# facebookresearch/omni3d

Measured on AMD Instinct MI355X. Metric: images/sec train DLA34_FPN b=4/GPU, higher is better.
Workload: dtype f32; 1 GPU; cubercnn_DLA34_FPN train step, batch 4/GPU, synthetic Omni3D 512x512 (8 GT/img), fwd+10 losses+bwd+allreduce+divergence guard+SGD, random-init weights; global_batch=4, image=512x512, parallelism=dp1 (flat-bucket RCCL all-reduce)

## Files before the change

### include/omni3d_hip.h

```cpp
#ifndef OMNI3D_HIP_H
#define OMNI3D_HIP_H

#ifdef __cplusplus
extern "C" {
#endif


int omni_iou_box3d(const float* boxes1, int N, const float* boxes2, int M, const int* valid1, float* vol,
                   float* iou, int* overflow, void* stream);

int omni_iou_box3d_pairs(const float* boxes1, const float* boxes2, const int* idx1, const int* idx2,
                         long long npairs, const int* valid1, float* vol, float* iou, int* overflow,
                         void* stream);

int omni_iou_box3d_pairs_algo(const float* boxes1, const float* boxes2, const int* idx1, const int* idx2,
                              long long npairs, const int* valid1, float* vol, float* iou, int* overflow,
                              int lanes_per_pair, void* stream);

int omni_box3d_validity(const float* boxes, int N, float eps_coplanar, float eps_nonzero, int* valid,
                        int* counts, void* stream);

int omni_nms3d(const float* verts, const float* score, const int* cls, const int* count, int B, int S, float iou_thr,
               int class_agnostic, float eps_coplanar, float eps_nonzero, float* iou, int* keep, int* order, int* new_count,
               int* overflow, void* stream);
// ... 102 lines not shown
                              int pad, int groups, void* stream);

int omni_dwconv_fwd(const float* x, const float* w, float* y, int N, int H, int W, int C, int R, int stride, int pad, void* stream);
int omni_dwconv_dgrad(const float* dy, const float* w, float* dx, int N, int H, int W, int C, int R, int stride, int pad, void* stream);
int omni_dwconv_wgrad(const float* x, const float* dy, float* dw, int N, int H, int W, int C, int R, int stride, int pad, void* stream);

int omni_avgpool2_fwd(const float* x, float* y, int N, int H, int W, int C, void* stream);
int omni_avgpool2_bwd(const float* dy, float* dx, int N, int H, int W, int C, void* stream);

int omni_subsample2_fwd(const float* x, float* y, int N, int H, int W, int C, void* stream);
int omni_subsample2_bwd(const float* dy, float* dx, int N, int H, int W, int C, void* stream);

int omni_upsample2_add(const float* lat, const float* top, float* out, int N, int H, int W, int C,
                       void* stream);
int omni_upsample2_bwd(const float* dout, float* dtop, int N, int H, int W, int C, void* stream);

int omni_wino_out_carry(const float* M, const float* carry, long long ldc, float* y, int N, int H, int W, int K, int tile, void* stream);
int omni_maxpool2_bwd_carry(const float* x, const float* dy, long long lddy, const float* carry, long long ldc, float* dx, int N, int H,
                            int W, int C, void* stream);
int omni_subsample2_bwd_carry(const float* dy, const float* carry, long long ldc, float* dx, int N, int H, int W, int C, void* stream);
int omni_upsample2_bwd_carry(const float* dout, const float* carry, long long ldc, float* dtop, int N, int H, int W, int C,
                             void* stream);

int omni_preprocess(const unsigned char* img, float* out, int N, int H, int W, int PH, int PW, float m0,
                    float m1, float m2, float s0, float s1, float s2, void* stream);
int omni_preprocess_masked(const unsigned char* img, const int* image_hw, float* out, int N, int H, int W, int PH, int PW,
                           float m0, float m1, float m2, float s0, float s1, float s2, void* stream);
int omni_preprocess_multi(const void* const* imgs, const int* image_hw, float* out, int N, int H, int W, int PH, int PW, float m0,
                          float m1, float m2, float s0, float s1, float s2, void* stream);

// ... 300 lines not shown
```

### omni3d_amd/csrc/conv_gemm.hip

```cpp
#include <device_rt.h>
#include "split_reduce.h"

namespace {

constexpr int OMNI_MAX_SRC = 6;
struct ConvP {
    const float* x;
    const float* w;
    const float* bias;
    float* out;
    int N, H, W, C;
    int OH, OW, K;
    int R, S, stride, pad;
    int ldx, ldo, ldw;
    int relu;
    int accumulate;
    int splits;
    long xb, wb, ob;
    float* stats;
    float* ws;
    unsigned* ctr;
    const float* xs[OMNI_MAX_SRC];
    int coff[OMNI_MAX_SRC + 1];
    int nsrc;
};


__device__ __forceinline__ float4 ldg4(const float* p) { return *reinterpret_cast<const float4*>(p); }
__device__ __forceinline__ float4 zero4() { return make_float4(0.f, 0.f, 0.f, 0.f); }
typedef unsigned omni_u4 __attribute__((ext_vector_type(4)));
__device__ __forceinline__ float4 bufld4(omni_rsrc_t r, int voff) {
#ifdef OMNI_HIPEMU
    float4 v = zero4();
    if ((unsigned)voff + 16u <= r.bytes) memcpy(&v, r.base + (unsigned)voff, 16);
    return v;
#else
    const omni_u4 u = __builtin_amdgcn_raw_buffer_load_b128(r, voff, 0, 0);
    return make_float4(__uint_as_float(u.x), __uint_as_float(u.y), __uint_as_float(u.z), __uint_as_float(u.w));
#endif
}


__device__ __forceinline__ void tile_coords(int tiles_m, int tiles_n, int& tm, int& tn) {
    const int nwg = tiles_m * tiles_n;
    int id = blockIdx.x;
    const int q = nwg / 8, r = nwg % 8;
    const int xcd = id % 8, k = id / 8;
    const int swz = (xcd < r ? xcd * (q + 1) : r * (q + 1) + (xcd - r) * q) + k;
    id = (nwg >= 8) ? swz : id;
    if (tiles_n <= 4) {
        tn = id % tiles_n;
        tm = id / tiles_n;
    } else {
        tm = id % tiles_m;
        tn = id / tiles_m;
    }
}

__device__ __forceinline__ int xcd_chunked(int id, int total) {
    if (total < 8) return id;
    const int q = total / 8, r = total % 8, xcd = id % 8, k = id / 8;
    return (xcd < r ? xcd * (q + 1) : r * (q + 1) + (xcd - r) * q) + k;
}

template <int WM, int WN, bool A_KCONTIG, bool B_KCONTIG, int LDA, int LDB, int BKX = 16>
__device__ __forceinline__ void mma_slab(const float* __restrict__ As, const float* __restrict__ Bs, int a_row0,
                                         int b_row0, int lane, f32x16 (&acc)[WM][WN]) {
    const int l31 = lane & 31, h = lane >> 5;
    constexpr int BKP = BKX + 4;
#pragma unroll
    for (int kc = 0; kc < BKX / 8; ++kc) {
        float a[WM][4], b[WN][4];
#pragma unroll
        for (int i = 0; i < WM; ++i) {
            if (A_KCONTIG) {
                const float4 v = *reinterpret_cast<const float4*>(As + (a_row0 + 32 * i + l31) * BKP + 8 * kc + 4 * h);
                a[i][0] = v.x; a[i][1] = v.y; a[i][2] = v.z; a[i][3] = v.w;
            } else {
#pragma unroll
                for (int t = 0; t < 4; ++t) a[i][t] = As[(8 * kc + 4 * h + t) * LDA + a_row0 + 32 * i + l31];
            }
        }
#pragma unroll
        for (int j = 0; j < WN; ++j) {
            if (B_KCONTIG) {
                const float4 v = *reinterpret_cast<const float4*>(Bs + (b_row0 + 32 * j + l31) * BKP + 8 * kc + 4 * h);
                b[j][0] = v.x; b[j][1] = v.y; b[j][2] = v.z; b[j][3] = v.w;
            } else {
#pragma unroll
                for (int t = 0; t < 4; ++t) b[j][t] = Bs[(8 * kc + 4 * h + t) * LDB + b_row0 + 32 * j + l31];
            }
        }
#pragma unroll
        for (int t = 0; t < 4; ++t)
#pragma unroll
            for (int i = 0; i < WM; ++i)
#pragma unroll
                for (int j = 0; j < WN; ++j) acc[i][j] = mfma_32x32x2(a[i][t], b[j][t], acc[i][j]);
    }
}

template <int WM, int WN>
__device__ __forceinline__ void zero_acc(f32x16 (&acc)[WM][WN]) {
#pragma unroll
    for (int i = 0; i < WM; ++i)
#pragma unroll
        for (int j = 0; j < WN; ++j)
#pragma unroll
            for (int r = 0; r < 16; ++r) acc[i][j][r] = 0.f;
}

template <int BM, int BN, int WAVES_M, int WAVES_N, int BKX = 16, int PF = 1>
__global__ void __launch_bounds__(256) conv_fwd_kernel(ConvP p) {
    constexpr int WM = BM / (32 * WAVES_M), WN = BN / (32 * WAVES_N);
    constexpr int BKP = BKX + 4, KQ = BKX / 4;
    constexpr int RPP = 256 / KQ;
    constexpr int AI = (BM + RPP - 1) / RPP, BI = (BN + RPP - 1) / RPP;
    __shared__ __attribute__((aligned(16))) float smem[2 * (BM + BN) * BKP];
    p.x += (long)blockIdx.z * p.xb;
    p.w += (long)blockIdx.z * p.wb;
    p.out += (long)blockIdx.z * p.ob;
    const int tid = threadIdx.x, lane = tid & 63, wave = tid >> 6;
    const int wm = wave / WAVES_N, wn = wave % WAVES_N;
    const int M = p.N * p.OH * p.OW, Kd = p.R * p.S * p.C;
// ... 934 lines not shown
    const int local = id - t.first[j];
    if (local >= t.items[j]) return;
    gemm_tn_pf_body<PF>(t.p[j], t.rps[j], t.splits[j], xcd_chunked(local, t.items[j]));
}

inline bool bad_geom(const ConvP& p) {
    return p.N < 0 || p.H <= 0 || p.W <= 0 || p.C <= 0 || p.K <= 0 || p.R <= 0 || p.S <= 0 || p.stride <= 0 ||
           p.pad < 0 || (p.C & 3) || p.OH != (p.H + 2 * p.pad - p.R) / p.stride + 1 ||
           p.OW != (p.W + 2 * p.pad - p.S) / p.stride + 1;
}

}

extern "C" {


struct DetArgs {
    float* ws;
    long long ws_floats;
    unsigned* ctr;
    int n_ctr;
    long long* plan;
};
constexpr DetArgs NO_DET{};
static inline bool det_fits(const DetArgs& d, long tiles, long splits, long tile_elems) {
    return d.ctr != nullptr && d.ws != nullptr && d.n_ctr >= omni_split_counters(tiles, splits) &&
           d.ws_floats >= omni_split_ws_floats(tiles, splits, tile_elems);
}
static inline void det_plan(const DetArgs& d, long tile, long tiles, long splits, long tile_elems) {
    d.plan[0] = tile; d.plan[1] = splits;
// ... 103 lines not shown
    ConvP p = convp_fwd(x, w, bias, out, N, H, W, C, K, R, S, stride, pad, ldx, ldo, relu);
    if (nblk_out) *nblk_out = 0;
    if (ms != nullptr && attach_sources(p, *ms, 32, true) != OMNI_OK) return OMNI_ERR_ARG;
    if (bad_geom(p) || (ldx & 3) || ldx < C || ldo < K || tile < 0 || tile > 4 || splits_req < 0) return OMNI_ERR_ARG;
    if (splits_req > 1 && ldo != K) return OMNI_ERR_ARG;
    const long M = (long)N * p.OH * p.OW;
    if (M == 0) return OMNI_OK;
    hipStream_t st = (hipStream_t)stream;
    const long Kd = (long)R * S * C;
    if (ms == nullptr && !fits_i32(((long)N * H * W - 1) * ldx + C)) return OMNI_ERR_ARG;
    if (!fits_i32((long)K * Kd)) return OMNI_ERR_ARG;
    const long nslab = (Kd + 31) / 32;
    const long t128 = ((M + 127) / 128) * ((K + 127) / 128);
    const long t64 = ((M + 63) / 64) * ((K + 63) / 64);
    long splits = 1;
    if (tile == 0) {
        if (K > 64 && t128 >= 256) {
            tile = 1;
        } else if (K > 64 && t128 >= 64 && Kd >= 2048 && ldo == K) {
            tile = 1;
            splits = (512 + t128 - 1) / t128;
            if (splits > nslab / 8) splits = nslab / 8;
        } else if (K > 32 && (K > 64 || ((M + 127) / 128) < 256)) {
            tile = 2;
            if (t64 < 512 && nslab >= 16 && ldo == K) {
                splits = (1024 + t64 - 1) / t64;
                if (splits > nslab / 8) splits = nslab / 8;
                if (splits > 32) splits = 32;
            }
        } else {
            tile = K > 32 ? 3 : 4;
        }
        if (splits < 1) splits = 1;
    }
    if (splits_req >= 1) splits = splits_req;
    if (splits > nslab) splits = nslab;
    int bm, bn;
    tile_dims(tile, bm, bn);
    const long tiles = ((M + bm - 1) / bm) * ((K + bn - 1) / bn);
    const DetLaunch dl = det_prologue(det, tile, tiles, splits, (long)bm * bn, out, sizeof(float) * (size_t)M * K, false, st);
    if (dl.step != DET_LAUNCH) return dl.step;
    p.ws = dl.ws; p.ctr = dl.ctr;
    if (stats != nullptr && (splits == 1 || dl.ordered) && bias == nullptr && !relu) {
        const long rows = (M + bm - 1) / bm;
        if (rows <= stats_rows) {
            p.stats = stats;
            if (nblk_out) *nblk_out = (int)rows;
        }
    }
#define OMNI_FWD(BM_, BN_, WM_, WN_, BK_, PF_)                                                                           \
    hipLaunchKernelGGL(HIP_KERNEL_NAME(conv_fwd_kernel<BM_, BN_, WM_, WN_, BK_, PF_>), dim3((unsigned)tiles, (unsigned)splits), dim3(256), 0, st, p)
// ... 46 lines not shown
static int conv2d_dgrad_impl(const float* dy, const float* w, float* dx, int N, int H, int W, int C, int K, int R, int S,
                             int stride, int pad, int lddy, int lddx, int accumulate, int tile, int splits_req, void* stream,
                             const DetArgs& det) {
    ConvP p = convp_dgrad(dy, w, dx, N, H, W, C, K, R, S, stride, pad, lddy, lddx, accumulate);
    if (bad_geom(p) || (K & 3) || (lddy & 3) || lddy < K || lddx < C || tile < 0 || tile > 4 || splits_req < 0) return OMNI_ERR_ARG;
    if (splits_req > 1 && lddx != C && !accumulate) return OMNI_ERR_ARG;
    if ((long)N * H * W == 0) return OMNI_OK;
    hipStream_t st = (hipStream_t)stream;
    const unsigned ncls = (unsigned)(stride * stride);
    const long M = (long)N * ((H + stride - 1) / stride) * ((W + stride - 1) / stride);
    const long Kd = (long)((R + stride - 1) / stride) * ((S + stride - 1) / stride) * K;
    const long nslab = (Kd + 31) / 32;
    const long t128 = ((M + 127) / 128) * ((C + 127) / 128);
    const long t64 = ((M + 63) / 64) * ((C + 63) / 64);
    long splits = 1;
    if (tile == 0) {
        if (C > 64 && t128 * ncls >= 256) {
            tile = 1;
        } else if (C > 32 && (C > 64 || ((M + 127) / 128) * ncls < 256)) {
            tile = 2;
            if (t64 * ncls < 512 && nslab >= 16 && (lddx == C || accumulate)) {
                splits = (1024 + t64 * ncls - 1) / (t64 * ncls);
                if (splits > nslab / 8) splits = nslab / 8;
                if (splits > 32) splits = 32;
                if (splits < 1) splits = 1;
            }
        } else {
            tile = C > 32 ? 3 : 4;
        }
    }
    if (splits_req >= 1) splits = splits_req;
    if (splits > nslab) splits = nslab;
    int bm, bn;
    tile_dims(tile, bm, bn);
    const long class_tiles = ((M + bm - 1) / bm) * ((C + bn - 1) / bn);
    const long tiles = class_tiles * ncls;
    const DetLaunch dl = det_prologue(det, tile, tiles, splits, (long)bm * bn, dx, sizeof(float) * (size_t)N * H * W * C, accumulate != 0, st);
    if (dl.step != DET_LAUNCH) return dl.step;
    p.ws = dl.ws; p.ctr = dl.ctr;
    const bool dpf = fits_i32((long)N * p.OH * p.OW * lddy, PF_HEADROOM) && fits_i32((long)K * R * S * C, PF_HEADROOM);
#define OMNI_DGRAD(BM_, BN_, WM_, WN_, BK_, PF_)                                                                         \
    hipLaunchKernelGGL(HIP_KERNEL_NAME(conv_dgrad_kernel<BM_, BN_, WM_, WN_, BK_, PF_>), dim3((unsigned)class_tiles, (unsigned)splits, ncls), dim3(256), 0, st, p)
    if (dpf && tile == 1) OMNI_DGRAD(128, 128, 2, 2, 32, 2);
    else if (dpf && tile == 2) OMNI_DGRAD(64, 64, 2, 2, 32, 2);
    else if (dpf && tile == 3) OMNI_DGRAD(128, 64, 2, 2, 32, 2);
    else if (tile == 1) OMNI_DGRAD(128, 128, 2, 2, 32, 1);
    else if (tile == 2) OMNI_DGRAD(64, 64, 2, 2, 32, 1);
// ... 295 lines not shown
```

### omni3d_amd/cubercnn/modeling/backbone/fpn.py

```python
import math

from torch import nn

from .... import functional as HF
from ....d2.layers import ShapeSpec
from ..layers import Conv2d


class Backbone(nn.Module):
    @property
    def size_divisibility(self):
        return 0

    def output_shape(self):
        return {name: ShapeSpec(channels=self._out_feature_channels[name], stride=self._out_feature_strides[name])
                for name in self._out_features}


class LastLevelMaxPool(nn.Module):

    def __init__(self):
        super().__init__()
        self.num_levels = 1
        self.in_feature = "p5"
# ... 29 lines not shown
            for s in range(stage, stage + top_block.num_levels):
                self._out_feature_strides[f"p{s + 1}"] = 2 ** (s + 1)
        self._out_features = list(self._out_feature_strides.keys())
        self._out_feature_channels = {k: out_channels for k in self._out_features}
        self._size_divisibility = strides[-1]

    @property
    def size_divisibility(self):
        return self._size_divisibility

    def forward(self, x):
        feats = self.bottom_up(x)
        results = {}
        prev = None
        for f, stage in zip(reversed(self.in_features), reversed(self._stages)):
            lat = getattr(self, f"fpn_lateral{stage}")(feats[f])
            prev = lat if prev is None else HF.upsample2_add(lat, prev)
            HF.fanout(prev)
            results[f"p{stage}"] = HF.fanout(getattr(self, f"fpn_output{stage}")(prev))
        if self.top_block is not None:
            src = feats[self.top_block.in_feature] if self.top_block.in_feature in feats else results[self.top_block.in_feature]
            for i, t in enumerate(self.top_block(src)):
                results[f"p{self._stages[-1] + 1 + i}"] = t
        return {k: results[k] for k in self._out_features}
```

### omni3d_amd/functional.py

```python
import torch
from torch.autograd import Function
from os import environ as _environ

_os_environ_get = _environ.get

from .kernels import glue
from .kernels import bnpool, conv, det, wino

CL = torch.channels_last


def _cl(t):
    return t if t.is_contiguous(memory_format=CL) else t.contiguous(memory_format=CL)


def _direct_grad(t):
    if t is not None and getattr(t, "_omni_direct_grad", False) and t.grad is not None and t.requires_grad:
        return t.grad
    return None


def _parts_out(parts, like):
    return parts if parts is not None else like.new_zeros((0, 1))

# ... 640 lines not shown
    def forward(ctx, lat, top):
        ctx.slot = _slot_enter(top, ctx.needs_input_grad[1])
        return bnpool.upsample2_add(_cl(lat), _cl(top))

    @staticmethod
    def backward(ctx, dout):
        dout = _cl(dout)

        def run(carry):
            if carry is not None and _carry_pitch(carry) is None:
                return bnpool.upsample2_bwd(dout) + carry
            return bnpool.upsample2_bwd(dout, carry=carry)
        return dout, _slot_deliver(ctx.slot, run)


class _CatChannels(Function):

    @staticmethod
    def forward(ctx, *xs):
        ctx.slots = [_slot_enter(x, ctx.needs_input_grad[i]) for i, x in enumerate(xs)]
        ctx.sizes = [x.shape[1] for x in xs]
        return torch.cat(xs, 1)

    @staticmethod
    def backward(ctx, g):
        outs, off = [], 0
        for i, (slot, c) in enumerate(zip(ctx.slots, ctx.sizes)):
            piece = g[:, off:off + c]
            off += c
            outs.append(_slot_deliver(slot, lambda carry, piece=piece: _add_carry(piece, carry)) if ctx.needs_input_grad[i] else None)
# ... 82 lines not shown

def max_pool2(x):
    return _MaxPool2.apply(x)


def avg_pool2(x):
    return _AvgPool2.apply(x)


def subsample2(x):
    return _Subsample2.apply(x)


def upsample2_add(lat, top):
    return _Upsample2Add.apply(lat, top)


def _pool_enter(ctx, k, feats):
    ctx.slots = [_slot_enter(f, ctx.needs_input_grad[k + i]) for i, f in enumerate(feats)]
    feats = [_cl(f) for f in feats]
    nhwc = [f.permute(0, 2, 3, 1) for f in feats]
    ctx.shapes = [tuple(f.shape) for f in nhwc]
    return nhwc


def _pool_deliver(ctx, k, dfe):
    return (None,) * k + tuple(_slot_deliver(slot, lambda carry, d=d: _add_carry(d.permute(0, 3, 1, 2), carry)) for slot, d in zip(ctx.slots, dfe))


class _ROIAlign(Function):
# ... 295 lines not shown
```

### omni3d_amd/kernels/conv.py

```python

import torch

from .. import lib as _lib
from . import detmode as _det


def _nhwc(t):
    if t.dim() != 4:
        raise ValueError("expected a 4-D tensor")
    v = t.permute(0, 2, 3, 1)
    if not v.is_contiguous():
        v = v.contiguous()
    return v


def to_channels_last(t):
    return t.contiguous(memory_format=torch.channels_last)


def _fwd_launch(L, x, w, bias, out, N, H, W, C, K, R, S, stride, pad, ldx, ldo, relu, tile, splits, like, stats=None, stats_rows=0, nblk_addr=None):
    if _det.on():
        _det.plan_launch(L, "omni_conv2d_fwd_det", like, (x, w, bias, out, N, H, W, C, K, R, S, stride, pad, ldx, ldo, int(relu)),
                         ask=(tile, splits), late=(_lib.ptr(stats), stats_rows, nblk_addr))
    elif stats is not None:
# ... 81 lines not shown
    n = len(xv)
    ptrs = (ctypes.c_void_p * n)(*[t.data_ptr() for t in xv])
    cs = (ctypes.c_int * n)(*[int(t.shape[3]) for t in xv])
    pa, ca = ctypes.cast(ptrs, ctypes.c_void_p), ctypes.cast(cs, ctypes.c_void_p)
    stats = _stats_buf(K, out.device) if want_stats and bias is None and not relu else None
    cell, addr = _nblk_cell()
    head = (pa, ca, n, _lib.ptr(wv), _lib.ptr(bias), _lib.ptr(out), N, H, W, K, K, int(relu))
    late = (_lib.ptr(stats), STATS_ROWS if stats is not None else 0, addr)
    if _det.on():
        _det.plan_launch(L, "omni_conv2d_fwd_multi_det", xv[0], head, ask=(tile, splits), late=late)
    else:
        L.call("omni_conv2d_fwd_multi_det", *head, tile, splits, *late, None, 0, None, 0, None, _lib.stream_of(xv[0]))
    return out.permute(0, 3, 1, 2), (stats[:cell.value] if stats is not None and cell.value > 0 else None)


def stem_conv_fwd_stats(x, w):
    xv, wv = _nhwc(x), _nhwc(w)
    N, H, W, C = xv.shape
    K, R = wv.shape[0], wv.shape[1]
    L = _lib.check_device(xv, wv)
    out = torch.empty((N, H, W, K), dtype=torch.float32, device=x.device)
    stats = _stats_buf(K, x.device)
    cell, addr = _nblk_cell()
    L.call("omni_stem_conv_fwd_stats", _lib.ptr(xv), _lib.ptr(wv), _lib.ptr(out), N, H, W, C, K, R, C, K, _lib.ptr(stats), STATS_ROWS, addr,
           _lib.stream_of(x))
    return out.permute(0, 3, 1, 2), (stats[:cell.value] if cell.value > 0 else None)


_S2_DGRAD_MIN_WGS = 192

# ... 292 lines not shown
```

### omni3d_amd/profile_io.py

```python
import csv
import hashlib
import os
import re

ROOT = os.path.dirname(os.path.dirname(os.path.abspath(__file__)))


def profile_counters(csv_name, kernel_substr, grid=None):
    path = os.path.join(ROOT, "profiles", csv_name)
    if not os.path.exists(path):
        return None
    digest = hashlib.sha256(open(path, "rb").read()).hexdigest()[:16]
    rows = [r for r in csv.DictReader(open(path)) if kernel_substr in r["kernel"] and (grid is None or int(float(r["grid"])) == grid)]
    if not rows:
        return None
    r = max(rows, key=lambda q: float(q.get("GRBM_GUI_ACTIVE", "0") or 0))

    def f(k):
        try:
            v = float(r[k])
            return v if v == v else None
        except (KeyError, ValueError):
            return None
    out = {"source": f"profiles/{csv_name}", "sha256_16": digest, "kernel": r["kernel"], "grid": int(float(r["grid"]))}
# ... 65 lines not shown
        return None
    if name in VALU_ENTRIES:
        return "valu"
    if name.startswith("omni_rpn_head16"):
        return "head16"
    if name.startswith("omni_stem_conv"):
        return "stem"
    if name.startswith("omni_gemm_engine"):
        return "engine"
    if name == "omni_gemm_batched_wgrad_multi":
        return "gemm_batched_multi"
    if name.startswith("omni_gemm_batched"):
        return "gemm_batched"
    if name.startswith("omni_grouped_conv2d"):
        return "grouped"
    if name in ("omni_conv2d_fwd_multi_det", "omni_conv2d_wgrad_multi_det"):
        return "conv_multi"
    if name == "omni_conv2d_s2_dgrad":
        return "conv_s2"
    if name.startswith("omni_conv2d"):
        return "conv"
    return None


def _host_ints(ptr, n, ctype):
    import ctypes
    if ptr is None:
        return []
    addr = ptr.value if hasattr(ptr, "value") else int(ptr)
    return list(ctypes.cast(addr, ctypes.POINTER(ctype))[:n])


def executed_flops(name, a):
    import ctypes
    cls = flop_class(name)
    if cls in (None, "valu"):
        return 0.0
    v = dict(zip(abi_signatures()[name], a))
    if v.get("plan") is not None:
        return 0.0
    if cls in ("conv", "grouped"):
        OH = (v["H"] + 2 * v["pad"] - v["R"]) // v["stride"] + 1
        OW = (v["W"] + 2 * v["pad"] - v["S"]) // v["stride"] + 1
        return 2.0 * v["N"] * OH * OW * v["K"] * v["R"] * v["S"] * v["C"] / (v["groups"] if cls == "grouped" else 1)
    if cls == "conv_multi":
        return 2.0 * v["N"] * v["H"] * v["W"] * v["K"] * sum(_host_ints(v["cs"], v["nsrc"], ctypes.c_int))
    if cls == "conv_s2":
        return 2.0 * v["N"] * ((v["H"] - 1) // 2 + 1) * ((v["W"] - 1) // 2 + 1) * v["K"] * 9 * v["C"]
    if cls == "stem":
        stride = 2 if "_s2_" in name else 1
        OH, OW = (v["H"] - 1) // stride + 1, (v["W"] - 1) // stride + 1
        return 2.0 * v["N"] * OH * OW * v["K"] * v["R"] * v["R"] * v["C"]
    if cls == "gemm_batched":
        if "N" in v and "C" not in v:
            return 2.0 * v["batch"] * v["M"] * v["N"] * v["K"]
        return 2.0 * v["batch"] * v["M"] * v["C"] * v["K"]
    if cls == "gemm_batched_multi":
        n = v["n"]
        cols = [_host_ints(v[k], n, ctypes.c_int) for k in ("batch", "M", "C", "K")]
        return float(sum(2.0 * b * m * c * k for b, m, c, k in zip(*cols)))
    if cls == "engine":
# ... 81 lines not shown
```

Baseline: 384.0 images/s.

## Add persistent pointwise 1x1 conv GEMM kernel and fuse FPN lateral with upsample-add

Adds a dedicated persistent 1x1-conv GEMM kernel that keeps the full weight slab in shared memory and streams pixel tiles, dispatched automatically for large-M 1x1 forward and dgrad convolutions. The FPN top-down path now fuses the lateral 1x1 conv with the nearest-upsample-and-add of the coarser level in one kernel's epilogue, removing an intermediate tensor write and read. Shared GEMM fragment helpers are moved into a header. The change risks being slower than the tuned generic conv GEMM for some shapes and adds new backward plumbing for the fused op.

```diff
diff --git a/include/omni3d_hip.h b/include/omni3d_hip.h
--- a/include/omni3d_hip.h
+++ b/include/omni3d_hip.h
@@ -140,6 +140,14 @@
 int omni_upsample2_add(const float* lat, const float* top, float* out, int N, int H, int W, int C,
                        void* stream);
 int omni_upsample2_bwd(const float* dout, float* dtop, int N, int H, int W, int C, void* stream);
+
+int omni_conv1x1_fwd_up2add(const float* x, const float* w, const float* bias, const float* top, float* out, int N,
+                            int H, int W, int C, int K, int ldx, int ldo, void* stream);
+int omni_conv1x1_fwd_algo(const void* const* xs, const int* cs, int nsrc, const float* w, const float* bias,
+                          const float* top, float* out, int N, int H, int W, int K, int ldx, int ldo, int relu,
+                          float* stats, int stats_rows, int* nblk_out, int workgroups, void* stream);
+int omni_conv1x1_dgrad_algo(const float* dy, const float* w, float* dx, int N, int H, int W, int C, int K, int lddy,
+                            int lddx, int accumulate, int workgroups, void* stream);
 
 int omni_wino_out_carry(const float* M, const float* carry, long long ldc, float* y, int N, int H, int W, int K, int tile, void* stream);
 int omni_maxpool2_bwd_carry(const float* x, const float* dy, long long lddy, const float* carry, long long ldc, float* dx, int N, int H,
diff --git a/omni3d_amd/csrc/conv_gemm.hip b/omni3d_amd/csrc/conv_gemm.hip
--- a/omni3d_amd/csrc/conv_gemm.hip
+++ b/omni3d_amd/csrc/conv_gemm.hip
@@ -1,5 +1,7 @@
 #include <device_rt.h>
+#include "gemm_frag.h"
 #include "split_reduce.h"
+#include "pointwise_plan.h"
 
 namespace {
 
@@ -26,21 +28,6 @@
 };
 
 
-__device__ __forceinline__ float4 ldg4(const float* p) { return *reinterpret_cast<const float4*>(p); }
-__device__ __forceinline__ float4 zero4() { return make_float4(0.f, 0.f, 0.f, 0.f); }
-typedef unsigned omni_u4 __attribute__((ext_vector_type(4)));
-__device__ __forceinline__ float4 bufld4(omni_rsrc_t r, int voff) {
-#ifdef OMNI_HIPEMU
-    float4 v = zero4();
-    if ((unsigned)voff + 16u <= r.bytes) memcpy(&v, r.base + (unsigned)voff, 16);
-    return v;
-#else
-    const omni_u4 u = __builtin_amdgcn_raw_buffer_load_b128(r, voff, 0, 0);
-    return make_float4(__uint_as_float(u.x), __uint_as_float(u.y), __uint_as_float(u.z), __uint_as_float(u.w));
-#endif
-}
-
-
 __device__ __forceinline__ void tile_coords(int tiles_m, int tiles_n, int& tm, int& tn) {
     const int nwg = tiles_m * tiles_n;
     int id = blockIdx.x;
@@ -55,59 +42,6 @@
         tm = id % tiles_m;
         tn = id / tiles_m;
     }
-}
-
-__device__ __forceinline__ int xcd_chunked(int id, int total) {
-    if (total < 8) return id;
-    const int q = total / 8, r = total % 8, xcd = id % 8, k = id / 8;
-    return (xcd < r ? xcd * (q + 1) : r * (q + 1) + (xcd - r) * q) + k;
-}
-
-template <int WM, int WN, bool A_KCONTIG, bool B_KCONTIG, int LDA, int LDB, int BKX = 16>
-__device__ __forceinline__ void mma_slab(const float* __restrict__ As, const float* __restrict__ Bs, int a_row0,
-                                         int b_row0, int lane, f32x16 (&acc)[WM][WN]) {
-    const int l31 = lane & 31, h = lane >> 5;
-    constexpr int BKP = BKX + 4;
-#pragma unroll
-    for (int kc = 0; kc < BKX / 8; ++kc) {
-        float a[WM][4], b[WN][4];
-#pragma unroll
-        for (int i = 0; i < WM; ++i) {
-            if (A_KCONTIG) {
-                const float4 v = *reinterpret_cast<const float4*>(As + (a_row0 + 32 * i + l31) * BKP + 8 * kc + 4 * h);
-                a[i][0] = v.x; a[i][1] = v.y; a[i][2] = v.z; a[i][3] = v.w;
-            } else {
-#pragma unroll
-                for (int t = 0; t < 4; ++t) a[i][t] = As[(8 * kc + 4 * h + t) * LDA + a_row0 + 32 * i + l31];
-            }
-        }
-#pragma unroll
-        for (int j = 0; j < WN; ++j) {
-            if (B_KCONTIG) {
-                const float4 v = *reinterpret_cast<const float4*>(Bs + (b_row0 + 32 * j + l31) * BKP + 8 * kc + 4 * h);
-                b[j][0] = v.x; b[j][1] = v.y; b[j][2] = v.z; b[j][3] = v.w;
-            } else {
-#pragma unroll
-                for (int t = 0; t < 4; ++t) b[j][t] = Bs[(8 * kc + 4 * h + t) * LDB + b_row0 + 32 * j + l31];
-            }
-        }
-#pragma unroll
-        for (int t = 0; t < 4; ++t)
-#pragma unroll
-            for (int i = 0; i < WM; ++i)
-#pragma unroll
-                for (int j = 0; j < WN; ++j) acc[i][j] = mfma_32x32x2(a[i][t], b[j][t], acc[i][j]);
-    }
-}
-
-template <int WM, int WN>
-__device__ __forceinline__ void zero_acc(f32x16 (&acc)[WM][WN]) {
-#pragma unroll
-    for (int i = 0; i < WM; ++i)
-#pragma unroll
-        for (int j = 0; j < WN; ++j)
-#pragma unroll
-            for (int r = 0; r < 16; ++r) acc[i][j][r] = 0.f;
 }
 
 template <int BM, int BN, int WAVES_M, int WAVES_N, int BKX = 16, int PF = 1>
@@ -1072,6 +1006,12 @@
 
 extern "C" {
 
+int omni_conv1x1_fwd_algo(const void* const* xs, const int* cs, int nsrc, const float* w, const float* bias, const float* top, float* out,
+                          int N, int H, int W, int K, int ldx, int ldo, int relu, float* stats, int stats_rows, int* nblk_out,
+                          int workgroups, void* stream);
+int omni_conv1x1_dgrad_algo(const float* dy, const float* w, float* dx, int N, int H, int W, int C, int K, int lddy, int lddx,
+                            int accumulate, int workgroups, void* stream);
+
 
 struct DetArgs {
     float* ws;
@@ -1205,6 +1145,7 @@
     const long t128 = ((M + 127) / 128) * ((K + 127) / 128);
     const long t64 = ((M + 63) / 64) * ((K + 63) / 64);
     long splits = 1;
+    const bool own_choice = tile == 0 && splits_req == 0;
     if (tile == 0) {
         if (K > 64 && t128 >= 256) {
             tile = 1;
@@ -1226,6 +1167,12 @@
     }
     if (splits_req >= 1) splits = splits_req;
     if (splits > nslab) splits = nslab;
+    if (own_choice && splits == 1 && det.plan == nullptr && R == 1 && S == 1 && stride == 1 && pad == 0 && stats == nullptr && ms == nullptr &&
+        pw_dispatch(M, C)) {
+        const void* xs1[1] = {x};
+        const int cs1[1] = {C};
+        return omni_conv1x1_fwd_algo(xs1, cs1, 1, w, bias, nullptr, out, N, H, W, K, ldx, ldo, relu, nullptr, 0, nullptr, 0, stream);
+    }
     int bm, bn;
     tile_dims(tile, bm, bn);
     const long tiles = ((M + bm - 1) / bm) * ((K + bn - 1) / bn);
@@ -1302,6 +1249,7 @@
     const long t128 = ((M + 127) / 128) * ((C + 127) / 128);
     const long t64 = ((M + 63) / 64) * ((C + 63) / 64);
     long splits = 1;
+    const bool own_choice = tile == 0 && splits_req == 0;
     if (tile == 0) {
         if (C > 64 && t128 * ncls >= 256) {
             tile = 1;
@@ -1319,6 +1267,8 @@
     }
     if (splits_req >= 1) splits = splits_req;
     if (splits > nslab) splits = nslab;
+    if (own_choice && splits == 1 && det.plan == nullptr && R == 1 && S == 1 && stride == 1 && pad == 0 && pw_dispatch(M, K))
+        return omni_conv1x1_dgrad_algo(dy, w, dx, N, H, W, C, K, lddy, lddx, accumulate, 0, stream);
     int bm, bn;
     tile_dims(tile, bm, bn);
     const long class_tiles = ((M + bm - 1) / bm) * ((C + bn - 1) / bn);
diff --git a/omni3d_amd/csrc/gemm_frag.h b/omni3d_amd/csrc/gemm_frag.h
--- /dev/null
+++ b/omni3d_amd/csrc/gemm_frag.h
@@ -0,0 +1,73 @@
+#pragma once
+#include <device_rt.h>
+
+namespace {
+
+__device__ __forceinline__ float4 ldg4(const float* p) { return *reinterpret_cast<const float4*>(p); }
+__device__ __forceinline__ float4 zero4() { return make_float4(0.f, 0.f, 0.f, 0.f); }
+typedef unsigned omni_u4 __attribute__((ext_vector_type(4)));
+__device__ __forceinline__ float4 bufld4(omni_rsrc_t r, int voff) {
+#ifdef OMNI_HIPEMU
+    float4 v = zero4();
+    if ((unsigned)voff + 16u <= r.bytes) memcpy(&v, r.base + (unsigned)voff, 16);
+    return v;
+#else
+    const omni_u4 u = __builtin_amdgcn_raw_buffer_load_b128(r, voff, 0, 0);
+    return make_float4(__uint_as_float(u.x), __uint_as_float(u.y), __uint_as_float(u.z), __uint_as_float(u.w));
+#endif
+}
+
+__device__ __forceinline__ int xcd_chunked(int id, int total) {
+    if (total < 8) return id;
+    const int q = total / 8, r = total % 8, xcd = id % 8, k = id / 8;
+    return (xcd < r ? xcd * (q + 1) : r * (q + 1) + (xcd - r) * q) + k;
+}
+
+template <int WM, int WN, bool A_KCONTIG, bool B_KCONTIG, int LDA, int LDB, int BKX = 16>
+__device__ __forceinline__ void mma_slab(const float* __restrict__ As, const float* __restrict__ Bs, int a_row0,
+                                         int b_row0, int lane, f32x16 (&acc)[WM][WN]) {
+    const int l31 = lane & 31, h = lane >> 5;
+    constexpr int BKP = BKX + 4;
+#pragma unroll
+    for (int kc = 0; kc < BKX / 8; ++kc) {
+        float a[WM][4], b[WN][4];
+#pragma unroll
+        for (int i = 0; i < WM; ++i) {
+            if (A_KCONTIG) {
+                const float4 v = *reinterpret_cast<const float4*>(As + (a_row0 + 32 * i + l31) * BKP + 8 * kc + 4 * h);
+                a[i][0] = v.x; a[i][1] = v.y; a[i][2] = v.z; a[i][3] = v.w;
+            } else {
+#pragma unroll
+                for (int t = 0; t < 4; ++t) a[i][t] = As[(8 * kc + 4 * h + t) * LDA + a_row0 + 32 * i + l31];
+            }
+        }
+#pragma unroll
+        for (int j = 0; j < WN; ++j) {
+            if (B_KCONTIG) {
+                const float4 v = *reinterpret_cast<const float4*>(Bs + (b_row0 + 32 * j + l31) * BKP + 8 * kc + 4 * h);
+                b[j][0] = v.x; b[j][1] = v.y; b[j][2] = v.z; b[j][3] = v.w;
+            } else {
+#pragma unroll
+                for (int t = 0; t < 4; ++t) b[j][t] = Bs[(8 * kc + 4 * h + t) * LDB + b_row0 + 32 * j + l31];
+            }
+        }
+#pragma unroll
+        for (int t = 0; t < 4; ++t)
+#pragma unroll
+            for (int i = 0; i < WM; ++i)
+#pragma unroll
+                for (int j = 0; j < WN; ++j) acc[i][j] = mfma_32x32x2(a[i][t], b[j][t], acc[i][j]);
+    }
+}
+
+template <int WM, int WN>
+__device__ __forceinline__ void zero_acc(f32x16 (&acc)[WM][WN]) {
+#pragma unroll
+    for (int i = 0; i < WM; ++i)
+#pragma unroll
+        for (int j = 0; j < WN; ++j)
+#pragma unroll
+            for (int r = 0; r < 16; ++r) acc[i][j][r] = 0.f;
+}
+
+}
diff --git a/omni3d_amd/csrc/pointwise.hip b/omni3d_amd/csrc/pointwise.hip
--- /dev/null
+++ b/omni3d_amd/csrc/pointwise.hip
@@ -0,0 +1,336 @@
+#include <device_rt.h>
+#include "gemm_frag.h"
+#include "pointwise_plan.h"
+
+namespace {
+
+constexpr int PW_MAX_SRC = 6;
+struct PwP {
+    const float* x;
+    const float* w;
+    const float* bias;
+    const float* top;
+    float* out;
+    float* stats;
+    int M, Rd, Nn;
+    int H, W;
+    int ldx, ldo;
+    int relu, dgrad, accumulate;
+    int nslab, ncg, tiles_m;
+    const float* xs[PW_MAX_SRC];
+    int coff[PW_MAX_SRC + 1];
+    int nsrc;
+};
+
+template <int BN, bool TR>
+__global__ void __launch_bounds__(PW_THREADS) pw_gemm_kernel(PwP p) {
+    constexpr int BKX = PW_BK, BKP = BKX + 4, KQ = BKX / 4, KC = BKX / 8, WN = BN / 32, NW = PW_THREADS / 64;
+    constexpr int PF = 2, JB = WN < 4 ? WN : 4;
+    __shared__ __attribute__((aligned(16))) float smem[PW_W_ROWS * BKP + NW * BN];
+    float* Wl = smem;
+    float* red = Wl + PW_W_ROWS * BKP;
+    const int tid = threadIdx.x, lane = tid & 63, wave = tid >> 6;
+    const int l31 = lane & 31, h = lane >> 5;
+    int cg, ri, t0, t1;
+    pw_item((int)blockIdx.x, (int)gridDim.x, p.ncg, cg, ri);
+    pw_range(p.tiles_m, (int)gridDim.x / p.ncg, ri, t0, t1);
+    if (t0 >= t1) return;
+    const int n0 = cg * BN, nslab = p.nslab;
+    const int rounds = (t1 - t0 + 1) / 2;
+
+    f32x4 ra[PF][KC];
+    int ld_tile = t0 + (wave >> 2), ld_slab = 0;
+    auto load_slab = [&](const int sg) {
+        const int c0 = ld_slab * BKX;
+        const float* src = p.x;
+        int pitch = p.ldx, lo = 0, width = p.Rd;
+        if (p.nsrc > 0) {
+            src = p.xs[0]; width = p.coff[1];
+#pragma unroll
+            for (int q = 1; q < PW_MAX_SRC; ++q)
+                if (q < p.nsrc && c0 >= p.coff[q]) { src = p.xs[q]; lo = p.coff[q]; width = p.coff[q + 1] - p.coff[q]; }
+            pitch = width;
+        }
+        const omni_rsrc_t rx_ = omni_make_rsrc(src, (unsigned)((((long)p.M - 1) * pitch + width) * 4));
+        const int m = ld_tile * PW_BM + (wave & 3) * 32 + l31;
+        const bool ok = ld_tile < t1 && m < p.M;
+        const int cl = c0 - lo + 4 * h;
+#pragma unroll
+        for (int kc = 0; kc < KC; ++kc) {
+            const float4 v = bufld4(rx_, (ok && cl + 8 * kc < width) ? (m * pitch + cl + 8 * kc) * 4 : OMNI_OOB);
+            ra[sg][kc][0] = v.x; ra[sg][kc][1] = v.y; ra[sg][kc][2] = v.z; ra[sg][kc][3] = v.w;
+        }
+        if (++ld_slab == nslab) { ld_slab = 0; ld_tile += 2; }
+    };
+#pragma unroll
+    for (int sg = 0; sg < PF; ++sg) load_slab(sg);
+
+    const omni_rsrc_t rw_ = omni_make_rsrc(p.w, (unsigned)((long)p.Nn * p.Rd * 4));
+    if (!p.dgrad) {
+        for (int idx = tid; idx < nslab * BN * KQ; idx += PW_THREADS) {
+            const int q = idx % KQ, row = (idx / KQ) % BN, s = idx / (KQ * BN);
+            const int n = n0 + row, r = s * BKX + q * 4;
+            const float4 v = bufld4(rw_, (n < p.Nn && r < p.Rd) ? (n * p.Rd + r) * 4 : OMNI_OOB);
+            *reinterpret_cast<float4*>(Wl + (s * BN + row) * BKP + q * 4) = v;
+        }
+    } else {
+        for (int idx = tid; idx < nslab * BKX * (BN / 4); idx += PW_THREADS) {
+            const int c4 = idx % (BN / 4), r = idx / (BN / 4);
+            const int n = n0 + 4 * c4;
+            const float4 v = bufld4(rw_, (n < p.Nn && r < p.Rd) ? (r * p.Nn + n) * 4 : OMNI_OOB);
+            float* d = Wl + ((r / BKX) * BN + 4 * c4) * BKP + (r % BKX);
+            d[0] = v.x; d[BKP] = v.y; d[2 * BKP] = v.z; d[3 * BKP] = v.w;
+        }
+    }
+    __syncthreads();
+
+    const int TH = p.H >> 1, TW = p.W >> 1;
+    f32x16 acc[1][WN];
+    auto epilogue = [&](const int tile) {
+        const bool live = tile < t1;
+        const int m0 = tile * PW_BM + (wave & 3) * 32;
+        if constexpr (TR) {
+            const int m = m0 + l31;
+            if (!live || m >= p.M) return;
+            float* o = p.out + (long)m * p.ldo;
+            const float* tp = o;
+            if (p.top != nullptr) {
+                const int img = m / (p.H * p.W), rem = m - img * (p.H * p.W);
+                const int ih = rem / p.W, iw = rem - ih * p.W;
+                tp = p.top + ((long)(img * TH + (ih >> 1)) * TW + (iw >> 1)) * p.Nn;
+            }
+            const bool addend = p.top != nullptr || (p.dgrad && p.accumulate);
+            float4 tv[WN][4];
+            if (addend) {
+#pragma unroll
+                for (int j = 0; j < WN; ++j)
+#pragma unroll
+                    for (int g = 0; g < 4; ++g) {
+                        const int n = n0 + 32 * j + 8 * g + 4 * h;
+                        tv[j][g] = n < p.Nn ? ldg4(tp + n) : zero4();
+                    }
+            }
+            OMNI_SCHED_FENCE();
+#pragma unroll
+            for (int j = 0; j < WN; ++j)
+#pragma unroll
+                for (int g = 0; g < 4; ++g) {
+                    const int n = n0 + 32 * j + 8 * g + 4 * h;
+                    if (n < p.Nn) {
+                        float4 v = make_float4(acc[0][j][4 * g], acc[0][j][4 * g + 1], acc[0][j][4 * g + 2], acc[0][j][4 * g + 3]);
+                        if (p.dgrad) {
+                            if (p.accumulate) { v.x = tv[j][g].x + v.x; v.y = tv[j][g].y + v.y; v.z = tv[j][g].z + v.z; v.w = tv[j][g].w + v.w; }
+                        } else {
+                            const float4 bv = p.bias != nullptr ? ldg4(p.bias + n) : zero4();
+                            v.x += bv.x; v.y += bv.y; v.z += bv.z; v.w += bv.w;
+                            if (p.top != nullptr) {
+                                v.x = v.x + tv[j][g].x; v.y = v.y + tv[j][g].y; v.z = v.z + tv[j][g].z; v.w = v.w + tv[j][g].w;
+                            }
+                            if (p.relu) { v.x = fmaxf(v.x, 0.f); v.y = fmaxf(v.y, 0.f); v.z = fmaxf(v.z, 0.f); v.w = fmaxf(v.w, 0.f); }
+                        }
+                        *reinterpret_cast<float4*>(o + n) = v;
+                    }
+                }
+            return;
+        }
+        if (p.stats != nullptr) {
+#pragma unroll
+            for (int which = 0; which < 2; ++which) {
+#pragma unroll
+                for (int j = 0; j < WN; ++j) {
+                    float sv = 0.f;
+#pragma unroll
+                    for (int r = 0; r < 16; ++r) {
+                        const int m = m0 + (r & 3) + 8 * (r >> 2) + 4 * h;
+                        const float v = (live && m < p.M) ? acc[0][j][r] : 0.f;
+                        sv += which ? v * v : v;
+                    }
+                    sv += __shfl_xor(sv, 32, 64);
+                    if (h == 0) red[wave * BN + j * 32 + l31] = sv;
+                }
+                __syncthreads();
+                for (int idx = tid; idx < 2 * BN; idx += PW_THREADS) {
+                    const int g = idx / BN, nl = idx - g * BN;
+                    float t = 0.f;
+#pragma unroll
+                    for (int wq = 0; wq < 4; ++wq) t += red[(4 * g + wq) * BN + nl];
+                    if (tile - (wave >> 2) + g < t1 && n0 + nl < p.Nn)
+                        p.stats[((long)(tile - (wave >> 2) + g) * 2 + which) * p.Nn + n0 + nl] = t;
+                }
+                __syncthreads();
+            }
+        }
+        if (!live) return;
+        float bv[WN];
+#pragma unroll
+        for (int j = 0; j < WN; ++j) {
+            const int n = n0 + j * 32 + l31;
+            bv[j] = (p.bias != nullptr && n < p.Nn) ? p.bias[n] : 0.f;
+        }
+        const bool addend = p.top != nullptr || (p.dgrad && p.accumulate);
+        float tv[WN][16];
+        if (addend) {
+#pragma unroll
+            for (int r = 0; r < 16; ++r) {
+                const int m = m0 + (r & 3) + 8 * (r >> 2) + 4 * h;
+                const float* tp = p.out + (long)m * p.ldo;
+                if (!p.dgrad) {
+                    const int mm = m < p.M ? m : 0;
+                    const int img = mm / (p.H * p.W), rem = mm - img * (p.H * p.W);
+                    const int ih = rem / p.W, iw = rem - ih * p.W;
+                    tp = p.top + ((long)(img * TH + (ih >> 1)) * TW + (iw >> 1)) * p.Nn;
+                }
+#pragma unroll
+                for (int j = 0; j < WN; ++j) {
+                    const int n = n0 + j * 32 + l31;
+                    tv[j][r] = (m < p.M && n < p.Nn) ? tp[n] : 0.f;
+                }
+            }
+        }
+        OMNI_SCHED_FENCE();
+#pragma unroll
+        for (int r = 0; r < 16; ++r) {
+            const int m = m0 + (r & 3) + 8 * (r >> 2) + 4 * h;
+            if (m < p.M) {
+                float* o = p.out + (long)m * p.ldo;
+#pragma unroll
+                for (int j = 0; j < WN; ++j) {
+                    const int n = n0 + j * 32 + l31;
+                    if (n < p.Nn) {
+                        if (p.dgrad) {
+                            o[n] = p.accumulate ? (tv[j][r] + acc[0][j][r]) : acc[0][j][r];
+                        } else {
+                            float v = acc[0][j][r] + bv[j];
+                            if (p.top != nullptr) v = v + tv[j][r];
+                            if (p.relu) v = fmaxf(v, 0.f);
+                            o[n] = v;
+                        }
+                    }
+                }
+            }
+        }
+    };
+
+    zero_acc<1, WN>(acc);
+    const int T = rounds * nslab;
+    int tile = t0 + (wave >> 2), s = 0;
+    for (int q0 = 0; q0 < T; q0 += PF) {
+#pragma unroll
+        for (int u = 0; u < PF; ++u) {
+            if (q0 + u < T) {
+                const float* Bs = Wl + s * BN * BKP;
+#pragma unroll
+                for (int kc = 0; kc < KC; ++kc)
+#pragma unroll
+                    for (int j0 = 0; j0 < WN; j0 += JB) {
+                        float b[JB][4];
+#pragma unroll
+                        for (int j = 0; j < JB; ++j) {
+                            const float4 v = *reinterpret_cast<const float4*>(Bs + (32 * (j0 + j) + l31) * BKP + 8 * kc + 4 * h);
+                            b[j][0] = v.x; b[j][1] = v.y; b[j][2] = v.z; b[j][3] = v.w;
+                        }
+#pragma unroll
+                        for (int t = 0; t < 4; ++t)
+#pragma unroll
+                            for (int j = 0; j < JB; ++j)
+                                acc[0][j0 + j] = TR ? mfma_32x32x2(b[j][t], ra[u][kc][t], acc[0][j0 + j]) : mfma_32x32x2(ra[u][kc][t], b[j][t], acc[0][j0 + j]);
+                    }
+                load_slab(u);
+                if (++s == nslab) {
+                    epilogue(tile);
+                    zero_acc<1, WN>(acc);
+                    s = 0;
+                    tile += 2;
+                }
+            }
+        }
+    }
+}
+
+int pw_launch(PwP& p, int workgroups, hipStream_t st) {
+    PwPlan pl;
+    if (!pw_plan(p.M, p.Rd, p.Nn, workgroups, pl)) return OMNI_ERR_ARG;
+    p.nslab = pl.nslab; p.ncg = pl.ncg; p.tiles_m = pl.tiles_m;
+    const auto al16 = [](const void* q) { return ((uintptr_t)q & 15) == 0; };
+    const bool tr = p.stats == nullptr && (p.Nn & 3) == 0 && (p.ldo & 3) == 0 && al16(p.out) && al16(p.top) && al16(p.bias);
+#define OMNI_PW(BN_, TR_) hipLaunchKernelGGL(HIP_KERNEL_NAME(pw_gemm_kernel<BN_, TR_>), dim3((unsigned)pl.grid), dim3(PW_THREADS), 0, st, p)
+    if (pl.bn == 128 && tr) OMNI_PW(128, true);
+    else if (pl.bn == 128) OMNI_PW(128, false);
+    else if (tr) OMNI_PW(64, true);
+    else OMNI_PW(64, false);
+#undef OMNI_PW
+    return omni_launch_status();
+}
+
+inline bool pw_fits(long elems) { return elems * 4 < (1L << 31); }
+
+}
+
+extern "C" {
+
+int omni_conv1x1_fwd_algo(const void* const* xs, const int* cs, int nsrc, const float* w, const float* bias, const float* top, float* out,
+                          int N, int H, int W, int K, int ldx, int ldo, int relu, float* stats, int stats_rows, int* nblk_out,
+                          int workgroups, void* stream) {
+    if (nblk_out) *nblk_out = 0;
+    if (xs == nullptr || cs == nullptr || nsrc < 1 || nsrc > PW_MAX_SRC || w == nullptr || out == nullptr) return OMNI_ERR_ARG;
+    if (N < 0 || H <= 0 || W <= 0 || K <= 0 || ldo < K || workgroups < 0) return OMNI_ERR_ARG;
+    PwP p{};
+    long C = 0;
+    for (int q = 0; q < PW_MAX_SRC; ++q) {
+        const bool live = q < nsrc;
+        if (live && (xs[q] == nullptr || cs[q] <= 0 || (cs[q] & 3) || (nsrc > 1 && (cs[q] % PW_BK) != 0))) return OMNI_ERR_ARG;
+        p.xs[q] = live ? (const float*)xs[q] : nullptr;
+        p.coff[q] = (int)C;
+        C += live ? cs[q] : 0;
+        if (C > (1 << 20)) return OMNI_ERR_ARG;
+    }
+    p.coff[PW_MAX_SRC] = (int)C;
+    for (int q = nsrc; q < PW_MAX_SRC; ++q) p.coff[q] = (int)C;
+    const long M = (long)N * H * W;
+    if (M == 0) return OMNI_OK;
+    if (nsrc == 1) {
+        if ((ldx & 3) || ldx < C) return OMNI_ERR_ARG;
+        if (!pw_fits((M - 1) * ldx + C)) return OMNI_ERR_ARG;
+    } else {
+        for (int q = 0; q < nsrc; ++q)
+            if (!pw_fits(M * cs[q])) return OMNI_ERR_ARG;
+    }
+    if (!pw_fits((long)K * C)) return OMNI_ERR_ARG;
+    if (top != nullptr && ((H & 1) || (W & 1) || relu)) return OMNI_ERR_ARG;
+    if (stats != nullptr && (bias != nullptr || relu || top != nullptr)) return OMNI_ERR_ARG;
+    p.x = p.xs[0]; p.w = w; p.bias = bias; p.top = top; p.out = out;
+    p.M = (int)M; p.Rd = (int)C; p.Nn = K; p.H = H; p.W = W;
+    p.ldx = nsrc == 1 ? ldx : (int)C; p.ldo = ldo; p.relu = relu;
+    p.nsrc = nsrc > 1 ? nsrc : 0;
+    PwPlan pl;
+    if (!pw_plan(M, p.Rd, p.Nn, workgroups, pl)) return OMNI_ERR_ARG;
+    if (stats != nullptr && pl.tiles_m <= stats_rows) {
+        p.stats = stats;
+        if (nblk_out) *nblk_out = pl.tiles_m;
+    }
+    return pw_launch(p, workgroups, (hipStream_t)stream);
+}
+
+int omni_conv1x1_fwd_up2add(const float* x, const float* w, const float* bias, const float* top, float* out, int N, int H, int W, int C,
+                            int K, int ldx, int ldo, void* stream) {
+    if (top == nullptr) return OMNI_ERR_ARG;
+    const void* xs[1] = {x};
+    const int cs[1] = {C};
+    return omni_conv1x1_fwd_algo(xs, cs, 1, w, bias, top, out, N, H, W, K, ldx, ldo, 0, nullptr, 0, nullptr, 0, stream);
+}
+
+int omni_conv1x1_dgrad_algo(const float* dy, const float* w, float* dx, int N, int H, int W, int C, int K, int lddy, int lddx,
+                            int accumulate, int workgroups, void* stream) {
+    if (dy == nullptr || w == nullptr || dx == nullptr || N < 0 || H <= 0 || W <= 0 || C <= 0 || K <= 0) return OMNI_ERR_ARG;
+    if ((C & 3) || (K & 3) || (lddy & 3) || lddy < K || lddx < C || workgroups < 0) return OMNI_ERR_ARG;
+    const long M = (long)N * H * W;
+    if (M == 0) return OMNI_OK;
+    if (!pw_fits((M - 1) * lddy + K) || !pw_fits((long)K * C)) return OMNI_ERR_ARG;
+    PwP p{};
+    p.x = dy; p.w = w; p.out = dx;
+    p.M = (int)M; p.Rd = K; p.Nn = C; p.H = H; p.W = W;
+    p.ldx = lddy; p.ldo = lddx; p.dgrad = 1; p.accumulate = accumulate;
+    return pw_launch(p, workgroups, (hipStream_t)stream);
+}
+
+}
diff --git a/omni3d_amd/csrc/pointwise_plan.h b/omni3d_amd/csrc/pointwise_plan.h
--- /dev/null
+++ b/omni3d_amd/csrc/pointwise_plan.h
@@ -0,0 +1,57 @@
+#pragma once
+
+#if !defined(__HIPCC__) && !defined(OMNI_HIPEMU) && !defined(__host__)
+#define __host__
+#define __device__
+#endif
+
+constexpr int PW_BM = 128;
+constexpr int PW_BK = 32;
+constexpr int PW_W_ROWS = 512;
+constexpr int PW_CUS = 256;
+constexpr int PW_THREADS = 512;
+
+struct PwPlan {
+    int bn;
+    int nslab;
+    int ncg;
+    int tiles_m;
+    int nr;
+    int grid;
+};
+
+inline bool pw_plan(long M, int Rd, int Nn, int workgroups, PwPlan& pl) {
+    if (M <= 0 || Rd <= 0 || Nn <= 0 || workgroups < 0 || M > (1L << 30)) return false;
+    pl.nslab = (Rd + PW_BK - 1) / PW_BK;
+    if (pl.nslab > PW_W_ROWS / 64) return false;
+    const int fit = pl.nslab <= 4 ? 128 : 64;
+    const int need = Nn <= 64 ? 64 : 128;
+    pl.bn = fit < need ? fit : need;
+    pl.ncg = (Nn + pl.bn - 1) / pl.bn;
+    pl.tiles_m = (int)((M + PW_BM - 1) / PW_BM);
+    long nr = (workgroups > 0 ? workgroups : PW_CUS) / pl.ncg;
+    if (nr < 1) nr = 1;
+    if (nr > pl.tiles_m) nr = pl.tiles_m;
+    pl.nr = (int)nr;
+    pl.grid = pl.nr * pl.ncg;
+    return true;
+}
+
+__host__ __device__ inline void pw_range(int tiles_m, int nr, int i, int& t0, int& t1) {
+    const int q = tiles_m / nr, rem = tiles_m % nr;
+    t0 = i * q + (i < rem ? i : rem);
+    t1 = t0 + q + (i < rem ? 1 : 0);
+}
+
+__host__ __device__ inline void pw_item(int g, int grid, int ncg, int& cg, int& ri) {
+    if (grid % (8 * ncg) == 0) {
+        const int xcd = g % 8, k = g / 8;
+        cg = k % ncg;
+        ri = (k / ncg) * 8 + xcd;
+    } else {
+        cg = g % ncg;
+        ri = g / ncg;
+    }
+}
+
+inline bool pw_dispatch(long M, int Rd) { return M >= 65536 && (Rd % PW_BK) == 0 && Rd / PW_BK <= PW_W_ROWS / 64; }
diff --git a/omni3d_amd/cubercnn/modeling/backbone/fpn.py b/omni3d_amd/cubercnn/modeling/backbone/fpn.py
--- a/omni3d_amd/cubercnn/modeling/backbone/fpn.py
+++ b/omni3d_amd/cubercnn/modeling/backbone/fpn.py
@@ -67,8 +67,12 @@
         results = {}
         prev = None
         for f, stage in zip(reversed(self.in_features), reversed(self._stages)):
-            lat = getattr(self, f"fpn_lateral{stage}")(feats[f])
-            prev = lat if prev is None else HF.upsample2_add(lat, prev)
+            lateral = getattr(self, f"fpn_lateral{stage}")
+            if prev is not None and HF.lateral_sum_eligible(feats[f], lateral.weight, prev):
+                prev = HF.lateral_sum(feats[f], lateral.weight, lateral.bias, prev)
+            else:
+                lat = lateral(feats[f])
+                prev = lat if prev is None else HF.upsample2_add(lat, prev)
             HF.fanout(prev)
             results[f"p{stage}"] = HF.fanout(getattr(self, f"fpn_output{stage}")(prev))
         if self.top_block is not None:
diff --git a/omni3d_amd/functional.py b/omni3d_amd/functional.py
--- a/omni3d_amd/functional.py
+++ b/omni3d_amd/functional.py
@@ -678,6 +678,32 @@
         return dout, _slot_deliver(ctx.slot, run)
 
 
+class _LateralSum(Function):
+
+    @staticmethod
+    def forward(ctx, x, w, bias, top):
+        ctx.direct = (_direct_grad(w), _direct_grad(bias))
+        ctx.slot = _slot_enter(x, ctx.needs_input_grad[0])
+        ctx.top_slot = _slot_enter(top, ctx.needs_input_grad[3])
+        x, w = _cl(x), _cl(w)
+        ctx.stem = False
+        ctx.save_for_backward(x, w, None)
+        ctx.cfg = (1, 0, False, bias is not None)
+        return conv.conv1x1_up2add(x, w, bias, _cl(top))
+
+    @staticmethod
+    def backward(ctx, dout):
+        dout = _cl(dout)
+
+        def run(carry):
+            if carry is not None and _carry_pitch(carry) is None:
+                return bnpool.upsample2_bwd(dout) + carry
+            return bnpool.upsample2_bwd(dout, carry=carry)
+        dtop = _slot_deliver(ctx.top_slot, run) if ctx.needs_input_grad[3] else None
+        dx, dw, db = _Conv2d.backward(ctx, dout)[:3]
+        return dx, dw, db, dtop
+
+
 class _CatChannels(Function):
 
     @staticmethod
@@ -790,6 +816,23 @@
 
 def upsample2_add(lat, top):
     return _Upsample2Add.apply(lat, top)
+
+
+def lateral_sum_eligible(x, w, top):
+    if x.dim() != 4 or w.dim() != 4 or tuple(w.shape[2:]) != (1, 1) or x.dtype != torch.float32:
+        return False
+    N, C, H, W = x.shape
+    K = w.shape[0]
+    if (H | W) & 1 or tuple(top.shape) != (N, K, H // 2, W // 2) or w.shape[1] != C or C % 32:
+        return False
+    return conv.conv1x1_served(C) and N * H * W >= LATERAL_SUM_MIN_PIXELS
+
+
+LATERAL_SUM_MIN_PIXELS = 16384
+
+
+def lateral_sum(x, w, bias, top):
+    return _LateralSum.apply(x, w, bias, top)
 
 
 def _pool_enter(ctx, k, feats):
diff --git a/omni3d_amd/kernels/conv.py b/omni3d_amd/kernels/conv.py
--- a/omni3d_amd/kernels/conv.py
+++ b/omni3d_amd/kernels/conv.py
@@ -119,6 +119,64 @@
     return out.permute(0, 3, 1, 2), (stats[:cell.value] if stats is not None and cell.value > 0 else None)
 
 
+PW_MAX_SLABS = 8
+
+
+def conv1x1_served(reduction):
+    return reduction % 4 == 0 and (reduction + 31) // 32 <= PW_MAX_SLABS
+
+
+def conv1x1_fwd(xs, w, bias=None, top=None, relu=False, want_stats=False, workgroups=0):
+    import ctypes
+    xs = list(xs) if isinstance(xs, (list, tuple)) else [xs]
+    xv = [_nhwc(x) for x in xs]
+    wv = _nhwc(w)
+    N, H, W, _ = xv[0].shape
+    K = wv.shape[0]
+    assert wv.shape[1] == 1 and wv.shape[2] == 1 and wv.shape[3] == sum(t.shape[3] for t in xv)
+    tv = _nhwc(top) if top is not None else None
+    assert tv is None or tuple(tv.shape) == (N, H // 2, W // 2, K)
+    L = _lib.check_device(*xv, wv, bias, tv)
+    out = torch.empty((N, H, W, K), dtype=torch.float32, device=xv[0].device)
+    n = len(xv)
+    ptrs = (ctypes.c_void_p * n)(*[t.data_ptr() for t in xv])
+    cs = (ctypes.c_int * n)(*[int(t.shape[3]) for t in xv])
+    stats = _stats_buf(K, out.device) if want_stats else None
+    cell, addr = _nblk_cell()
+    L.call("omni_conv1x1_fwd_algo", ctypes.cast(ptrs, ctypes.c_void_p), ctypes.cast(cs, ctypes.c_void_p), n, _lib.ptr(wv), _lib.ptr(bias),
+           _lib.ptr(tv), _lib.ptr(out), N, H, W, K, int(xv[0].shape[3]), K, int(relu), _lib.ptr(stats), STATS_ROWS if want_stats else 0, addr,
+           workgroups, _lib.stream_of(xv[0]))
+    y = out.permute(0, 3, 1, 2)
+    return (y, stats[:cell.value] if cell.value > 0 else None) if want_stats else y
+
+
+def conv1x1_up2add(x, w, bias, top):
+    xv, wv, tv = _nhwc(x), _nhwc(w), _nhwc(top)
+    N, H, W, C = xv.shape
+    K = wv.shape[0]
+    assert tuple(tv.shape) == (N, H // 2, W // 2, K) and H % 2 == 0 and W % 2 == 0
+    L = _lib.check_device(xv, wv, bias, tv)
+    out = torch.empty((N, H, W, K), dtype=torch.float32, device=x.device)
+    L.call("omni_conv1x1_fwd_up2add", _lib.ptr(xv), _lib.ptr(wv), _lib.ptr(bias), _lib.ptr(tv), _lib.ptr(out), N, H, W, C, K, C, K,
+           _lib.stream_of(x))
+    return out.permute(0, 3, 1, 2)
+
+
+def conv1x1_dgrad(dy, w, accum_into=None, workgroups=0):
+    dyv, wv = _nhwc(dy), _nhwc(w)
+    N, H, W, K = dyv.shape
+    C = wv.shape[3]
+    L = _lib.check_device(dyv, wv)
+    if accum_into is not None:
+        assert tuple(accum_into.shape) == (N, C, H, W) and accum_into.stride(1) == 1
+        L.call("omni_conv1x1_dgrad_algo", _lib.ptr(dyv), _lib.ptr(wv), accum_into.data_ptr(), N, H, W, C, K, K, accum_into.stride(3), 1,
+               workgroups, _lib.stream_of(dy))
+        return accum_into
+    dx = torch.empty((N, H, W, C), dtype=torch.float32, device=dy.device)
+    L.call("omni_conv1x1_dgrad_algo", _lib.ptr(dyv), _lib.ptr(wv), _lib.ptr(dx), N, H, W, C, K, K, C, 0, workgroups, _lib.stream_of(dy))
+    return dx.permute(0, 3, 1, 2)
+
+
 def stem_conv_fwd_stats(x, w):
     xv, wv = _nhwc(x), _nhwc(w)
     N, H, W, C = xv.shape
diff --git a/omni3d_amd/profile_io.py b/omni3d_amd/profile_io.py
--- a/omni3d_amd/profile_io.py
+++ b/omni3d_amd/profile_io.py
@@ -103,8 +103,10 @@
         return "gemm_batched"
     if name.startswith("omni_grouped_conv2d"):
         return "grouped"
-    if name in ("omni_conv2d_fwd_multi_det", "omni_conv2d_wgrad_multi_det"):
+    if name in ("omni_conv2d_fwd_multi_det", "omni_conv2d_wgrad_multi_det", "omni_conv1x1_fwd_algo"):
         return "conv_multi"
+    if name.startswith("omni_conv1x1"):
+        return "conv1x1"
     if name == "omni_conv2d_s2_dgrad":
         return "conv_s2"
     if name.startswith("omni_conv2d"):
@@ -134,6 +136,8 @@
         return 2.0 * v["N"] * OH * OW * v["K"] * v["R"] * v["S"] * v["C"] / (v["groups"] if cls == "grouped" else 1)
     if cls == "conv_multi":
         return 2.0 * v["N"] * v["H"] * v["W"] * v["K"] * sum(_host_ints(v["cs"], v["nsrc"], ctypes.c_int))
+    if cls == "conv1x1":
+        return 2.0 * v["N"] * v["H"] * v["W"] * v["K"] * v["C"]
     if cls == "conv_s2":
         return 2.0 * v["N"] * ((v["H"] - 1) // 2 + 1) * ((v["W"] - 1) // 2 + 1) * v["K"] * 9 * v["C"]
     if cls == "stem":
```

Measured after the change: 384.1 images/s (median of 2 runs). Within noise of the previous version (+0.0%).
